# snayfach/MicrobeCensus

Hardware: AMD Instinct MI355X
Metric: reads/sec searched vs marker DB + AGS abs-error, 150 bp @ 1/2/4/8 GPU (higher is better)
Workload: dtype u8/int32

## Files before the change

microbecensus_amd/csrc/k_translate_seg.h:

```cpp
#pragma once
#include "mc_hip_common.h"

#define MC_TS_THREADS 64
#define MC_TS_WAVES (MC_TS_THREADS / 64)
#define MC_TS_READS (MC_TS_THREADS / 6)
#define MC_TS_NLNF(FP) ((FP) + 2 > 24 ? (FP) + 2 : 24)
#define MC_TS_STRIDE(FP) (((((FP) + 76 + 3) >> 2) | 1) << 2)
#define MC_TS_STAGE(L) ((((MC_TS_READS * (L)) > MC_TS_WAVES * 1488 ? (MC_TS_READS * (L)) : MC_TS_WAVES * 1488) + 15) & ~15)

struct McSegWaveLds { unsigned long long best[64]; uint32_t pre[66]; uint32_t pre2[66]; uint32_t bq[64]; uint16_t off[64]; uint8_t n[64]; };
static_assert(sizeof(McHsp) == 48 && sizeof(McGapTask) % 4 == 0, "k_eval_seeds copies its staging buffers as 16- and 4-byte words");
static_assert(sizeof(McSegWaveLds) == 1488, "MC_TS_STAGE reserves 1488 bytes per wave");
#ifdef MC_EXP_TIMING
__device__ unsigned long long g_ts_acc[12], g_ts_cnt[12];
#define MC_TS_TICK(k) do { const unsigned long long now_ = __builtin_readcyclecounter(); if (lane == 0) { ts_acc_[tcat_] += now_ - tlast_; ts_acc_[12 + tcat_] += 1; } tlast_ = now_; tcat_ = (k); } while (0)
#define MC_TS_BEGIN(k) __shared__ unsigned long long ts_acc_[24]; if (lane < 24) ts_acc_[lane] = 0; mc_wave_sync(); unsigned long long tlast_ = __builtin_readcyclecounter(); int tcat_ = (k)
#define MC_TS_PARAMS , unsigned long long &tlast_, int &tcat_, unsigned long long *ts_acc_
#define MC_TS_ARGS , tlast_, tcat_, ts_acc_
#define MC_TS_END do { mc_wave_sync(); if (lane < 12) { atomicAdd(&g_ts_acc[lane], ts_acc_[lane]); atomicAdd(&g_ts_cnt[lane], ts_acc_[12 + lane]); } } while (0)
#else
#define MC_TS_TICK(k) do { } while (0)
#define MC_TS_BEGIN(k) do { } while (0)
#define MC_TS_PARAMS
#define MC_TS_ARGS
#define MC_TS_END do { } while (0)
#endif
#define MC_SEG_KEY_ONE 0xBFF0000000000000ull

__device__ __forceinline__ unsigned long long mc_seg_key(double x)
{
    const unsigned long long u = (unsigned long long)__double_as_longlong(x);
    return (u >> 63) ? ~u : (u | 0x8000000000000000ull);
}

__device__ __forceinline__ void mc_seg_wave(const double *lnf, const int32_t *fx, const uint64_t *__restrict__ segtab, uint8_t *prot, int n, bool act, const McSegWS ws, McSegWaveLds *WL,
                                         const uint8_t *lds0, int lane MC_TS_PARAMS)
{
    const int W = (n <= 11) ? 8 : 12;
    MC_TS_TICK(0);
    enum { POP = 0, SCAN = 1, WAIT = 2, DONE = 3 };
    int st = (act && W <= n) ? POP : DONE;
    McBits192 Flo, Fhi, lo, nhi, mk;
    mc_bits_clear(Flo); mc_bits_clear(Fhi); mc_bits_clear(lo); mc_bits_clear(nhi); mc_bits_clear(mk);
    if (st != DONE) {
        mc_seg_window_flags_rg(fx, prot, n, W, Flo, Fhi);
        if (!(Flo.a | Flo.b | Flo.c)) st = DONE;
    }
    int sp = 1, base = 0, m = 0, i = 0, lowlim = 0, loi = 0, hii = 0;
    bool any = false;
    if (st != DONE) ws.stk[0] = (int16_t)(uint16_t)(n << 8);
    const unsigned long long ltmask = (1ull << lane) - 1;
    for (;;) {
        MC_TS_TICK(1);
        while (st == POP || st == SCAN) {
            if (st == POP) {
                if (sp == 0) { st = DONE; break; }
                sp--;
                base = MC_SEG_START(ws.stk[sp]); m = MC_SEG_LEN(ws.stk[sp]);
                if (W > m) continue;
                lo = mc_seg_flags_of(Flo, base, m, W);
                i = mc_bits_next(lo, 0);
                if (i >= m) continue;
                nhi = mc_bits_andnot(mc_bits_low(m), mc_seg_flags_of(Fhi, base, m, W));
                lowlim = 0; st = SCAN;
            }
            loi = mc_bits_prev(nhi, i) + 1; if (loi < lowlim) loi = lowlim;
            hii = mc_bits_next(nhi, i) - 1; if (hii > m - 1) hii = m - 1;
            st = WAIT;
        }
        const unsigned long long req = __ballot(st == WAIT);
        MC_TS_TICK(2);
        if (req == 0) break;
        const int nreq = __popcll(req);
        const int myr = __popcll(req & ltmask);
        const int myn = hii - loi + 1;
        if (st == WAIT) {
            WL->off[myr] = (uint16_t)((prot + base + loi) - lds0);
            WL->n[myr] = (uint8_t)myn;
            WL->best[myr] = MC_SEG_KEY_ONE; WL->bq[myr] = 0xFFFFFFFFu;
        }
        mc_wave_sync();
#define MC_SEG_CJ(j, sh) (((((j) >> (sh)) * (((j) >> (sh)) + 1)) << (sh)) / 2 + ((j) & ((1 << (sh)) - 1)) * (((j) >> (sh)) + 1))
        int sh0 = 3, sh1 = 3;
        {
            int K = 0, j0 = 0;
            if (lane < nreq) { const int nn = WL->n[lane], minlen = (nn - 100 > 1) ? nn - 100 : 1; K = nn - minlen; j0 = nn - 15 > 0 ? (nn - 15 < K ? nn - 15 : K) : 0; }
            uint32_t s0 = 0, s1 = 0;
#pragma unroll
            for (int sh = 2; sh >= 0; sh--) {
                const uint32_t c1 = (uint32_t)MC_SEG_CJ(j0, sh), c0 = (uint32_t)MC_SEG_CJ(K, sh) - c1;
                const uint32_t t0 = (uint32_t)__builtin_amdgcn_readlane((int)mc_wave_scan_add(c0), 63), t1 = (uint32_t)__builtin_amdgcn_readlane((int)mc_wave_scan_add(c1), 63);
                if (t0 <= 64) sh0 = sh;
                if (t1 <= 64) sh1 = sh;
            }
            {
                const uint32_t c1 = sh1 == 0 ? (uint32_t)MC_SEG_CJ(j0, 0) : sh1 == 1 ? (uint32_t)MC_SEG_CJ(j0, 1) : sh1 == 2 ? (uint32_t)MC_SEG_CJ(j0, 2) : (uint32_t)MC_SEG_CJ(j0, 3);
                const uint32_t cj0 = sh0 == 0 ? (uint32_t)MC_SEG_CJ(j0, 0) : sh0 == 1 ? (uint32_t)MC_SEG_CJ(j0, 1) : sh0 == 2 ? (uint32_t)MC_SEG_CJ(j0, 2) : (uint32_t)MC_SEG_CJ(j0, 3);
                const uint32_t ck = sh0 == 0 ? (uint32_t)MC_SEG_CJ(K, 0) : sh0 == 1 ? (uint32_t)MC_SEG_CJ(K, 1) : sh0 == 2 ? (uint32_t)MC_SEG_CJ(K, 2) : (uint32_t)MC_SEG_CJ(K, 3);
                s0 = mc_wave_scan_add(ck - cj0); s1 = mc_wave_scan_add(c1);
            }
            if (lane == 0) { WL->pre[0] = 0; WL->pre2[0] = 0; }
            WL->pre[lane + 1] = s0; WL->pre2[lane + 1] = s1;
        }
        mc_wave_sync();
        for (int cls = 0; cls < 2; cls++) {
        const uint32_t *pre = cls ? WL->pre2 : WL->pre;
        const uint32_t total = pre[nreq];
        const int sh = cls ? sh1 : sh0, R = 1 << sh;
        for (uint32_t p0 = 0; p0 < total; p0 += 64) {
            MC_TS_TICK(3 + cls);
            const uint32_t p = p0 + (uint32_t)lane;
            const bool ok = p < total;
            int r = 0;
            for (int stp = 32; stp > 0; stp >>= 1) { const int k = r + stp; if (k < nreq && p >= pre[k]) r = k; }
            if (!ok) r = 0;
            const int nn = WL->n[r];
            int x = (int)(p - pre[r]);
            if (cls == 0) { const int minlen = (nn - 100 > 1) ? nn - 100 : 1, K = nn - minlen, j0 = nn - 15 > 0 ? (nn - 15 < K ? nn - 15 : K) : 0; x += MC_SEG_CJ(j0, sh); }
            int A = (int)((sqrtf(1.0f + 8.0f * (float)x / (float)R) - 1.0f) * 0.5f);
            while ((((A + 1) * (A + 2)) << sh) / 2 <= x) A++;
            while (((A * (A + 1)) << sh) / 2 > x) A--;
            const int rem = x - ((A * (A + 1)) << sh) / 2, B = rem / (A + 1), run = rem - B * (A + 1);
            const int j = (A << sh) + B, wfirst = run << sh, wlast = (wfirst + R - 1 < j) ? wfirst + R - 1 : j;
            const uint8_t *s = lds0 + WL->off[r];
            const int len = nn - j;
            const uint32_t qbase = (uint32_t)(j * (j + 1) / 2);
            unsigned long long key = MC_SEG_KEY_ONE;
            uint32_t kq = 0xFFFFFFFFu;
            if (ok) {
                if (cls == 0) {
                    McRhState rg; rg.clo = 0; rg.chi = 0; rg.hist = 0;
                    for (int k = 0; k < len; k++) mc_rh_add(rg, s[wfirst + k]);
                    const int cnt = wlast - wfirst + 1;
                    uint64_t svs[8];
#pragma unroll
                    for (int t = 0; t < 8; t++) {
                        svs[t] = rg.hist | ((uint64_t)len << 60);
                        if (t + 1 < cnt) { mc_rh_remove(rg, s[wfirst + t]); mc_rh_add(rg, s[wfirst + t + len]); }
                    }
#pragma unroll
                    for (int t0 = 0; t0 < 8; t0 += 4) {
                        if (t0 && R <= 4) break;
                        ulonglong2 ea[4], eb[4];
#pragma unroll
                        for (int t = 0; t < 4; t++) {
// ... 28 lines not shown
            mc_wave_sync();
            const unsigned long long nb = WL->best[r];
            if (ok && nb != old) WL->bq[r] = 0xFFFFFFFFu;
            mc_wave_sync();
            if (cand && key == nb) atomicMin(&WL->bq[r], kq);
            mc_wave_sync();
        }
        }
#undef MC_SEG_CJ
        MC_TS_TICK(6);
        if (st == WAIT) {
            const uint32_t q = WL->bq[myr];
            int lend = 0, rend = myn - 1;
            if (q != 0xFFFFFFFFu) {
                int j = (int)((sqrtf((float)(8u * q + 1u)) - 1.0f) * 0.5f);
                while ((uint32_t)((j + 1) * (j + 2) / 2) <= q) j++;
                while ((uint32_t)(j * (j + 1) / 2) > q) j--;
                const int len = myn - j, w0 = (int)q - j * (j + 1) / 2;
                lend = w0; rend = len + w0 - 1;
            }
            const int leftend = loi + lend, rightend = hii - (myn - rend - 1);
            if (i < leftend) {
                const int l2 = loi, r2 = leftend - 1;
                sp = mc_seg_push(ws.stk, sp, W, base + l2, r2 - l2 + 1);
            }
            mk = mc_bits_or(mk, mc_bits_range(base + leftend, base + rightend));
            any = true;
            lowlim = ((hii < rightend) ? hii : rightend) + 1;
            i = mc_bits_next(lo, lowlim);
            st = i < m ? SCAN : POP;
        }
        mc_wave_sync();
    }
    MC_TS_TICK(7);
    if (any) for (int k = 0; k < n; k++) if (mc_bits_test(mk, k)) prot[k] = MC_INV;
    MC_TS_TICK(10);
}

__device__ __forceinline__ int mc_translate_frame_lds(const uint8_t *cod, const uint8_t *read, int len, int frame, uint8_t *prot)
{
    const int o = frame % 3;
    int n = (len - o) / 3;
    if (n < 0) n = 0;
    const bool rc = frame >= 3;
    const uint32_t set = rc ? MC_NT_RC_SET : MC_NT_FWD_SET, perm = rc ? MC_NT_RC_PERM : MC_NT_FWD_PERM;
    const uint8_t *p = read + (rc ? len - 1 - o : o);
    const int s = rc ? -1 : 1;
    int i = 0;
    for (; i + 8 <= n; i += 8) {
        uint32_t b[24], w[2] = {0, 0};
#pragma unroll
        for (int k = 0; k < 24; k++) b[k] = p[s * (3 * i + k)];
#pragma unroll
        for (int k = 0; k < 8; k++) {
            const int a0 = mc_nt_code(b[3 * k], set, perm), a1 = mc_nt_code(b[3 * k + 1], set, perm), a2 = mc_nt_code(b[3 * k + 2], set, perm);
            const uint32_t aa = cod[(16 * a0 + 4 * a1 + a2) & 63];
            w[k >> 2] |= ((a0 | a1 | a2) < 0 ? (uint32_t)MC_INV : aa) << (8 * (k & 3));
        }
        *(uint32_t *)(prot + i) = w[0];
        *(uint32_t *)(prot + i + 4) = w[1];
    }
    for (; i < n; i++) {
        const int a0 = mc_nt_code(p[s * (3 * i)], set, perm), a1 = mc_nt_code(p[s * (3 * i + 1)], set, perm), a2 = mc_nt_code(p[s * (3 * i + 2)], set, perm);
        const uint8_t aa = cod[(16 * a0 + 4 * a1 + a2) & 63];
        prot[i] = (a0 | a1 | a2) < 0 ? (uint8_t)MC_INV : aa;
    }
    return n;
}

template <bool STAGED>
__global__ void __attribute__((amdgpu_waves_per_eu(4, 4))) __launch_bounds__(MC_TS_THREADS) k_translate_seg(const McTables *__restrict__ T, const uint8_t *__restrict__ reads, int L,
                                                       int64_t nreads, uint8_t *__restrict__ frames, int FP, const uint64_t *__restrict__ segtab)
{
    extern __shared__ __attribute__((aligned(16))) uint8_t smem[];
    const int tid = threadIdx.x;
    const int64_t r0 = (int64_t)blockIdx.x * MC_TS_READS;
    const int nr = (int)((nreads - r0) < MC_TS_READS ? (nreads - r0) : MC_TS_READS);
    const int rbytes = nr * L;
    const int stride = MC_TS_STRIDE(FP);
    __shared__ int32_t fxs[64];
#ifdef MC_EXP_TIMING
    const int lane = mc_lane();
#endif
    MC_TS_BEGIN(8);
    uint8_t *sreads = smem;
    const int nlnf = MC_TS_NLNF(FP);
    double *lnf = (double *)(smem + (STAGED ? MC_TS_STAGE(L) : MC_TS_STAGE(0)));
    uint8_t *rows = (uint8_t *)(lnf + nlnf);
    __shared__ __attribute__((aligned(4))) uint8_t cod[64];
    if (tid < 64) fxs[tid] = T->seg_dout[tid];
    if (tid < 16) ((uint32_t *)cod)[tid] = ((const uint32_t *)T->codon)[tid];
    for (int i = tid; i < nlnf; i += MC_TS_THREADS) lnf[i] = T->lnfac[i];
    if (STAGED) {
        const uint8_t *src = reads + r0 * L;
        const int head = (int)((4 - ((uintptr_t)src & 3)) & 3), nhead = head < rbytes ? head : rbytes;
        if (tid < nhead) sreads[tid] = src[tid];
        const int nw = (rbytes - nhead) >> 2;
        if (nhead == 0) for (int i = tid; i < nw; i += MC_TS_THREADS) ((uint32_t *)sreads)[i] = ((const uint32_t *)src)[i];
        else for (int i = tid; i < nw; i += MC_TS_THREADS) { const uint32_t w = ((const uint32_t *)(src + nhead))[i]; uint8_t *d = sreads + nhead + 4 * i; d[0] = (uint8_t)w; d[1] = (uint8_t)(w >> 8); d[2] = (uint8_t)(w >> 16); d[3] = (uint8_t)(w >> 24); }
        for (int i = nhead + 4 * nw + tid; i < rbytes; i += MC_TS_THREADS) sreads[i] = src[i];
    }
    __syncthreads();
    MC_TS_TICK(9);
    const int lr = tid / 6, f = tid - lr * 6;
    uint8_t *prot = rows + (size_t)tid * stride;
    int n = 0;
    if (lr < nr) n = mc_translate_frame_lds(cod, STAGED ? sreads + lr * L : reads + (r0 + lr) * L, L, f, prot);
    __syncthreads();
    {
        McSegWS ws; ws.comp = prot + FP; ws.sv = prot + FP + 20; ws.stk = (int16_t *)(prot + FP + 44);
        mc_seg_wave(lnf, fxs, segtab, prot, n, lr < nr, ws, (McSegWaveLds *)smem + (tid >> 6), rows, mc_lane() MC_TS_ARGS);
        if (lr < nr) for (int i = n; i < FP; i++) prot[i] = MC_INV;
    }
    __syncthreads();
    {
        uint32_t *dst = (uint32_t *)(frames + r0 * 6 * FP);
        const int total = nr * 6 * FP / 4, fpw = FP / 4;
        for (int i = tid; i < total; i += MC_TS_THREADS) { const int row = i / fpw, col = i - row * fpw; dst[i] = *(const uint32_t *)(rows + (size_t)row * stride + 4 * col); }
    }
    MC_TS_TICK(0);
    MC_TS_END;
}
```

microbecensus_amd/csrc/mc_hip.hip:

```cpp
#include "mc_hip_common.h"
#include "k_translate_seg.h"
#include "k_enumerate.h"
#include "k_eval_seeds.h"
#include "k_gapped.h"
#include "k_order.h"
#include "k_finish.h"
#include "k_grid.h"
#include "k_simulate.h"
#include "k_community.h"
#include "k_varlen.h"
#include "k_classes.h"
#include "k_bootstrap.h"
#include "k_wfit.h"
#include "mc_pieces.h"
#include "mc_ahead.h"
#include "mc_owned.h"
#include "mc_abund.h"

#include <map>

struct McCtx {
    McStream stream; hipStream_t side = nullptr, side2 = nullptr;
    McEvent ev[8], ev_fork, ev_join, ev_join2;
    int64_t cap_reads = 0; int pool_len = 0;
    int ts_staged = -1;
    uint32_t cap_tasks = 0, cap_gaps = 0, cap_hsps = 0, cap_rows = 0;
    McDev<uint8_t> d_frames_base; uint8_t *d_frames = nullptr;
    McDev<unsigned long long> d_stats;
    McDev<McSeedTask> d_tasks; McDev<McGapTask> d_gaps; McDev<McHsp> d_hsps, d_v, d_tmp;
    McDev<uint64_t> d_k64, d_hkeys, d_hplace, d_places; McDev<uint32_t> d_idx, d_idxo, d_heads, d_scan, d_gsz, d_nv, d_ghist;
    McDev<uint32_t> d_counters;
    McDev<McRow> d_rows; McDev<uint32_t> d_nrow, d_rowoff; McDev<McBestHit> d_best, d_bestof; McDev<uint8_t> d_low, d_cand;
    McDev<McGapCell> d_gws_full; McDev<uint32_t> d_retry, d_retry2; int gap_threads_full = 0;
    McDev<unsigned long long> d_gtab; uint32_t gtab_slots = 0; McDev<uint32_t> d_gleader; McDev<McFlankOut> d_fout;
    McPin<uint32_t> h_c; McPin<unsigned long long> h_stats; McPin<McBestHit> h_best; size_t h_best_cap = 0;
    const uint8_t *reads = nullptr; int64_t n = 0, first_read_id = 0, first = 0;
    int ahead_from = -1;
    bool own_a0 = true;
    uint32_t ntasks = 0, ngaps = 0, gpad = 0, nh = 0, nh_all = 0, nheads = 0, nrows = 0, nbest = 0, nsegs = 0;
    bool busy = false;
};

struct mc_handle {
    McHostIndex H;
    std::vector<int32_t> fam;
    int nfam = 0, device = 0;
    McDev<uint8_t> d_res_base; uint8_t *d_res = nullptr; McDev<uint32_t> d_off, d_bstart, d_post; McDev<unsigned long long> d_post8; McDev<uint16_t> d_keys; McDev<int32_t> d_fam;
    McDev<McTables> d_T; McDev<McClassPars> d_P;
    McTables hT; McClassPars hP;
    int read_len = 0, FP = 0; bool run_set = false;
    McDev<uint32_t> d_bitmap;
    McDev<McBucketRec> d_rec;
    McDev<uint32_t> d_filt, d_wild, d_pair; McDev<uint64_t> d_segtab; McDev<unsigned long long> d_rt;
    bool fast_enum = false;
    bool count_traffic = false;
    int pipe_nout = 0;
    bool keep_rows = true;
    bool best_only = false;
    bool rows_stay = false;
    float train_ms[3] = {0, 0, 0};
// ... 291 lines not shown
    const int newFP = ((read_len / 3 + 2) + 3) & ~3;
    if (newFP != h->FP || read_len != h->read_len) h->ctx.cap_reads = 0;
    h->read_len = read_len; h->FP = newFP; h->run_set = true;
    h->cls_set = false;
    MC_OT("set_run: segtab, uploads", t0);
    return 0;
}

static void best_materialize(mc_handle *h);
static int ensure_capacity(mc_handle *h, McCtx &c, int64_t nreads)
{
    if (nreads <= c.cap_reads && h->read_len <= c.pool_len) return 0;
    if (h->best_from == &c) best_materialize(h);
    ahead_drop(h);
    double t0 = mc_now();
    int64_t cap = nreads;
    if (cap > (1 << 21) - 1) { g_err = "batch larger than 2097151 reads"; return -1; }
    const int64_t L = h->read_len;
    c.cap_reads = 0;
    c.cap_tasks = (uint32_t)std::min<int64_t>(cap * (L + 32) + (1 << 20) + (int64_t)256 * 32 * MC_EN_BLK, 0x7fffffff);
    const int64_t ev_pad = (int64_t)256 * 8 * (MC_EV_BS / 64) * MC_EV_BLK;
    c.cap_gaps = (uint32_t)std::min<int64_t>(cap * (L / 8 + 8) + (1 << 18) + ev_pad, (1 << 27) - 2);
    c.cap_hsps = (uint32_t)std::min<int64_t>(cap * (L / 3 + 8) + (1 << 20) + ev_pad, 0x7fffffff);
    c.cap_rows = (uint32_t)std::min<int64_t>(cap * 16 + (1 << 20), 0x7fffffff);
    c.gap_threads_full = 16 * 1024;
    if (c.d_frames_base.alloc((size_t)cap * 6 * h->FP + 128) || c.d_tasks.alloc(c.cap_tasks) ||
        c.d_gaps.alloc(c.cap_gaps) || c.d_hsps.alloc(c.cap_hsps) || c.d_v.alloc(c.cap_hsps) ||
        c.d_tmp.alloc((size_t)c.cap_hsps * 2) || c.d_k64.alloc(c.cap_hsps) || c.d_hkeys.alloc(c.cap_hsps) || c.d_hplace.alloc(c.cap_hsps) || c.d_places.alloc(c.cap_hsps) || c.d_idx.alloc(c.cap_hsps) ||
        c.d_idxo.alloc(c.cap_hsps) || c.d_heads.alloc((size_t)cap + 2) || c.d_scan.alloc((size_t)4100) || c.d_gsz.alloc(c.cap_hsps) || c.d_nv.alloc((size_t)cap + 1) || c.d_rows.alloc(c.cap_rows) ||
        c.d_low.alloc((size_t)cap + 64) || c.d_cand.alloc((size_t)cap + 64) || c.d_nrow.alloc((size_t)cap + 1) || c.d_rowoff.alloc((size_t)cap + 1) || c.d_best.alloc((size_t)cap + 1) || c.d_bestof.alloc((size_t)cap + 1) ||
        c.d_gws_full.alloc((size_t)c.gap_threads_full * MC_GAP_W) || c.d_retry.alloc((size_t)c.cap_gaps * 2 + (size_t)cap + 1) || c.d_retry2.alloc((size_t)c.cap_gaps * 2) || c.d_gleader.alloc((size_t)c.cap_gaps) ||
        c.d_fout.alloc((size_t)c.cap_gaps * 2))
        return -1;
    c.d_frames = c.d_frames_base + 64;
    HIPCK(hipMemsetAsync(c.d_frames_base, MC_INV, 64, c.stream));
    if (c.h_best.alloc((size_t)cap + 1)) return -1;
    c.h_best_cap = (size_t)cap + 1;
    c.cap_reads = cap; c.pool_len = (int)L;
    HIPCK(hipStreamSynchronize(c.stream));
    MC_OT("ensure_capacity (pools)", t0);
    return 0;
}

static int reads_reserve(mc_handle *h, int64_t nreads)
{
    const int64_t need = nreads * (int64_t)h->read_len + 16;
    if (need > h->cap_own) { reads_change(h); if (h->d_reads.alloc((size_t)need)) return -1; h->cap_own = need; }
    return 0;
}

extern "C" int mc_upload(mc_handle *h, const uint8_t *reads, int64_t nreads)
{
    if (!h || !h->run_set) { g_err = "mc_set_run() must be called first"; return -1; }
    HIPCK(hipSetDevice(h->device));
    reads_change(h);
    if (reads_reserve(h, nreads)) return -1;
    if (nreads) HIPCK(hipMemcpyAsync(h->d_reads, reads, (size_t)nreads * h->read_len, hipMemcpyHostToDevice, h->ctx.stream));
    HIPCK(hipStreamSynchronize(h->ctx.stream));
    h->reads_dev = h->d_reads; h->nreads = nreads;
    return 0;
}

extern "C" int mc_attach(mc_handle *h, const void *device_reads, int64_t nreads)
{
    if (!h || !h->run_set) { g_err = "mc_set_run() must be called first"; return -1; }
    reads_change(h);
    h->reads_dev = (const uint8_t *)device_reads; h->nreads = nreads;
    return 0;
}

static int stage_wait(McCtx &c) { HIPCK(hipStreamSynchronize(c.stream)); return 0; }
static int counters_to_host(McCtx &c) { HIPCK(hipMemcpyAsync(c.h_c, c.d_counters, sizeof(uint32_t) * C_N, hipMemcpyDeviceToHost, c.stream)); return 0; }

#ifdef MC_EXP_TIMING
static int exp_timing_dump(mc_handle *h, McCtx &c, char stage)
{
    ahead_drop(h);
    if (stage == 'a') {
        HIPCK(hipStreamSynchronize(c.stream));
        unsigned long long acc[12], cnt[12];
        HIPCK(hipMemcpyFromSymbol(acc, HIP_SYMBOL(g_ts_acc), sizeof acc)); HIPCK(hipMemcpyFromSymbol(cnt, HIP_SYMBOL(g_ts_cnt), sizeof cnt));
        const char *nm[12] = {"flags", "advance", "numbering", "class-0 rounds", "class-1 rounds", "reduction", "owners", "mask", "staging", "translation", "write-out", ""};
        const double waves = (double)((c.n + MC_TS_READS - 1) / MC_TS_READS) * MC_TS_WAVES;
        for (int k = 0; k < 11; k++) fprintf(stderr, "ts-timing %-15s %9.1f cycles/wave  %8.2f entries/wave  total %8.1f Mcycles\n", nm[k], (double)acc[k] / waves, (double)cnt[k] / waves, acc[k] / 1e6);
        unsigned long long z[12] = {0, 0, 0, 0, 0, 0, 0, 0, 0, 0, 0, 0};
        HIPCK(hipMemcpyToSymbol(HIP_SYMBOL(g_ts_acc), z, sizeof z)); HIPCK(hipMemcpyToSymbol(HIP_SYMBOL(g_ts_cnt), z, sizeof z));
    } else {
        HIPCK(hipStreamSynchronize(c.stream)); HIPCK(hipStreamSynchronize(c.side));
        unsigned long long acc[8], cnt[8];
        HIPCK(hipMemcpyFromSymbol(acc, HIP_SYMBOL(g_fh_acc), sizeof acc)); HIPCK(hipMemcpyFromSymbol(cnt, HIP_SYMBOL(g_fh_cnt), sizeof cnt));
        {
            unsigned long long fr[8];
            HIPCK(hipMemcpyFromSymbol(fr, HIP_SYMBOL(g_fr_acc), sizeof fr));
            const char *fn[7] = {"groups", "items", "std::sort", "threshold, keys", "heap sort", "rows", "classification"};
            for (int k = 0; k < 7; k++) fprintf(stderr, "fr-timing %-17s total %9.1f Mcycles (thread wall time, summed)\n", fn[k], fr[k] / 1e6);
            unsigned long long z8[8] = {0, 0, 0, 0, 0, 0, 0, 0};
            HIPCK(hipMemcpyToSymbol(HIP_SYMBOL(g_fr_acc), z8, sizeof z8));
            HIPCK(hipMemcpyFromSymbol(fr, HIP_SYMBOL(g_fr_acc2), sizeof fr));
            const char *gn[8] = {"-", "sort by frame", "sort by start, stable", "choice", "sum statistics", "copies", "groups (count)", "groups linked (count)"};
            for (int k = 1; k < 8; k++) fprintf(stderr, "fg-timing %-22s %12.1f M\n", gn[k], fr[k] / 1e6);
            HIPCK(hipMemcpyToSymbol(HIP_SYMBOL(g_fr_acc2), z8, sizeof z8));
        }
        {
            unsigned long long ev[8];
            HIPCK(hipMemcpyFromSymbol(ev, HIP_SYMBOL(g_ev_acc), sizeof ev));
            const char *en[7] = {"loop, records asked", "survivors queued", "X-drop extension", "HSP, marks", "records written", "residue wait + seed", "growth, gate"};
            for (int k = 0; k < 7; k++) fprintf(stderr, "ev-timing %-21s total %9.1f Mcycles (lane 0 of every wave)\n", en[k], ev[k] / 1e6);
            unsigned long long z8[8] = {0, 0, 0, 0, 0, 0, 0, 0};
            HIPCK(hipMemcpyToSymbol(HIP_SYMBOL(g_ev_acc), z8, sizeof z8));
            unsigned long long tr[4];
            HIPCK(hipMemcpyFromSymbol(tr, HIP_SYMBOL(g_ev_turns), sizeof tr));
            fprintf(stderr, "ev-turns forward: %.1f M lane-turns in %.2f M wave-turns = %.1f lanes of 64; backward: %.1f M in %.2f M = %.1f lanes\n", tr[0] / 1e6, tr[1] / 1e6, tr[1] ? (double)tr[0] / (double)tr[1] : 0.0,
                    tr[2] / 1e6, tr[3] / 1e6, tr[3] ? (double)tr[2] / (double)tr[3] : 0.0);
            HIPCK(hipMemcpyToSymbol(HIP_SYMBOL(g_ev_turns), z8, sizeof tr));
        }
        const char *nm[8] = {"group starts", "groups", "scan, items", "sort", "threshold, ranks", "heap sort", "rows", "other"};
        for (int k = 0; k < 8; k++) fprintf(stderr, "fh-timing %-17s total %9.1f Mcycles %9llu entries\n", nm[k], acc[k] / 1e6, cnt[k]);
        {
            unsigned long long w[12];
            HIPCK(hipMemcpyFromSymbol(w, HIP_SYMBOL(g_fh_worst), sizeof w));
            fprintf(stderr, "fh-worst read: %llu stacked HSPs, %.3f Mcycles:", w[0] & 0xFFFFF, (double)(w[0] >> 20) / 1e6);
            for (int k = 0; k < 8; k++) fprintf(stderr, " %s %.3f", nm[k], (double)w[1 + k] / 1e6);
            fprintf(stderr, "\n");
            unsigned long long z12[12] = {0, 0, 0, 0, 0, 0, 0, 0, 0, 0, 0, 0};
            HIPCK(hipMemcpyToSymbol(HIP_SYMBOL(g_fh_worst), z12, sizeof z12));
        }
        unsigned long long z[8] = {0, 0, 0, 0, 0, 0, 0, 0};
        HIPCK(hipMemcpyToSymbol(HIP_SYMBOL(g_fh_acc), z, sizeof z)); HIPCK(hipMemcpyToSymbol(HIP_SYMBOL(g_fh_cnt), z, sizeof z));
    }
    return 0;
}
#else
static int exp_timing_dump(mc_handle *, McCtx &, char) { return 0; }
#endif

static int stage_a0(mc_handle *h, McCtx &c, hipStream_t st, const uint8_t *reads, int64_t at, int64_t n, hipEvent_t e0, hipEvent_t e1)
{
    const int L = h->read_len, FP = h->FP;
    uint8_t *frames = c.d_frames + at * 6 * FP;
    HIPCK(hipEventRecord(e0, st));
    const size_t lds_rest = (size_t)MC_TS_NLNF(FP) * 8 + (size_t)MC_TS_THREADS * MC_TS_STRIDE(FP);
    const size_t lds_staged = (size_t)MC_TS_STAGE(L) + lds_rest, lds_direct = (size_t)MC_TS_STAGE(0) + lds_rest;
    static const int ts_force = getenv("MC_TS_STAGED") ? atoi(getenv("MC_TS_STAGED")) : -1;
    const size_t cu_lds = 160 * 1024 - 1024;
    const bool staged = ts_force >= 0 ? ts_force != 0 : cu_lds / lds_staged >= cu_lds / lds_direct;
    const size_t lds = staged ? lds_staged : lds_direct;
    c.ts_staged = staged ? 1 : 0;
    const unsigned ts_blocks = (unsigned)((n + MC_TS_READS - 1) / MC_TS_READS);
    if (staged) {
        if (lds > 48 * 1024) HIPCK(hipFuncSetAttribute((const void *)k_translate_seg<true>, hipFuncAttributeMaxDynamicSharedMemorySize, (int)lds));
        k_translate_seg<true><<<dim3(ts_blocks), dim3(MC_TS_THREADS), lds, st>>>(h->d_T, reads, L, n, frames, FP, h->d_segtab);
    } else {
        if (lds > 48 * 1024) HIPCK(hipFuncSetAttribute((const void *)k_translate_seg<false>, hipFuncAttributeMaxDynamicSharedMemorySize, (int)lds));
        k_translate_seg<false><<<dim3(ts_blocks), dim3(MC_TS_THREADS), lds, st>>>(h->d_T, reads, L, n, frames, FP, h->d_segtab);
    }
    HIPCK(hipEventRecord(e1, st));
    return 0;
}

static int stage_a(mc_handle *h, McCtx &c, int64_t covered)
{
    const int64_t n = c.n;
    const int L = h->read_len, FP = h->FP;
    hipStream_t st = c.stream;
    McIndex X = dev_index(h);
    c.ntasks = c.ngaps = c.gpad = c.nh = c.nheads = c.nrows = c.nbest = c.nsegs = 0;
    HIPCK(hipMemsetAsync(c.d_counters, 0, sizeof(uint32_t) * C_N, st));
    HIPCK(hipMemsetAsync(c.d_stats, 0, sizeof(unsigned long long) * S_N, st));
    if (h->best_only) HIPCK(hipMemsetAsync(c.d_cand, 0, (size_t)n, st));
    HIPCK(hipMemsetAsync(c.d_low, 0, (size_t)n, st));
    c.own_a0 = covered < n;
    if (!c.own_a0) HIPCK(hipEventRecord(c.ev[1], st));
    else if (stage_a0(h, c, st, c.reads + covered * L, covered, n - covered, c.ev[0], c.ev[1])) return -1;
    if (exp_timing_dump(h, c, 'a')) return -1;
    const int64_t threads = n * 6;
    if (h->fast_enum) {
        const bool enq = !h->count_traffic;
        const size_t per_wave = enq ? MC_ENQ_WAVE_LDS(FP, L) : sizeof(McEnWave) + MC_EN_WAVE_LDS(FP, L);
        int waves = 0, bpc = 1;
        {
            static const int shapes_q[][2] = {{8, 2}, {4, 4}, {16, 1}, {12, 1}, {4, 3}, {8, 1}, {4, 2}, {4, 1}};
            static const int shapes_c[][2] = {{12, 2}, {8, 3}, {4, 6}, {4, 5}, {16, 1}, {8, 2}, {4, 4}, {12, 1}, {4, 3}, {8, 1}, {4, 2}, {4, 1}};
            if (enq) { for (const auto &sh : shapes_q) if (!waves && (size_t)sh[1] * (64 + sh[0] * per_wave) <= 160 * 1024) { waves = sh[0]; bpc = sh[1]; } }
            else for (const auto &sh : shapes_c) if (!waves && (size_t)sh[1] * (64 + sh[0] * per_wave) <= 160 * 1024) { waves = sh[0]; bpc = sh[1]; }
        }
        if (!waves) { g_err = "reads too long for the seed kernel's LDS layout"; return -1; }
        const size_t lds2 = 64 + waves * per_wave;
#define MC_LAUNCH_EN(KERNEL, WV)                                                                                                                   \
// ... 309 lines not shown

extern "C" int mc_range_begin(mc_handle *h, int64_t first, int64_t count, int64_t first_read_id)
{
    if (range_check(h, first, count)) return -1;
    if (count <= 0) { g_err = "mc_range_begin: an empty range"; return -1; }
    if (h->pipe_nout) { g_err = "mc_range_begin: a range is in flight already (mc_range_end first)"; return -1; }
    const int rc = range_begin(h, h->ctx, first, count, first_read_id);
    if (rc) return rc;
    h->pipe_nout = 1;
    return 0;
}

static int range_end_next(mc_handle *h, int64_t first, int64_t count, bool predict)
{
    if (predict) count = mc_ahead_predict(h->ctx.first, h->ctx.n, h->nreads, &first);
    return range_end(h, h->ctx, first, count);
}

extern "C" int64_t mc_ranges_translated_ahead(const mc_handle *h) { return h ? h->ahead_used : 0; }

extern "C" int mc_range_end(mc_handle *h)
{
    if (!h) { g_err = "null handle"; return -1; }
    if (h->pipe_nout == 0) { g_err = "mc_range_end: no range in flight"; return -1; }
    HIPCK(hipSetDevice(h->device));
    h->pipe_nout = 0;
    return range_end_next(h, 0, 0, true);
}

extern "C" int mc_ranges_in_flight(const mc_handle *h) { return h ? h->pipe_nout : 0; }

extern "C" int64_t mc_debug_stage(mc_handle *h, int what, void *dst, int64_t cap_bytes, int32_t *record_bytes)
{
    if (!h || !h->run_set || what < 0 || what > 5) { g_err = "mc_debug_stage: bad argument"; return -1; }
    if (h->pipe_nout) { g_err = "mc_debug_stage: ranges are in flight"; return -1; }
    HIPCK(hipSetDevice(h->device));
    ahead_drop(h);
    const McCtx &c = h->ctx;
    if (what == 4) {
        if (!c.h_c) { g_err = "mc_debug_stage: no range has run"; return -1; }
        const uint32_t v[3] = {c.h_c[C_ITEMS], c.h_c[C_RETRY], c.h_c[C_RETRY2]};
        if (record_bytes) *record_bytes = (int32_t)sizeof(uint32_t);
        if (dst && (int64_t)sizeof v <= cap_bytes) memcpy(dst, v, sizeof v);
        return (int64_t)sizeof v;
    }
    if (what == 5) {
        if (c.ts_staged < 0) { g_err = "mc_debug_stage: no range has run"; return -1; }
        const uint32_t v = (uint32_t)c.ts_staged;
        if (record_bytes) *record_bytes = (int32_t)sizeof v;
        if (dst && (int64_t)sizeof v <= cap_bytes) memcpy(dst, &v, sizeof v);
        return (int64_t)sizeof v;
    }
    const void *src = nullptr; int64_t bytes = 0; int32_t rec = 0;
    if (what == 0) { src = c.d_frames; rec = h->FP; bytes = c.n * 6 * (int64_t)h->FP; }
    else if (what == 1) { src = c.d_tasks; rec = (int32_t)sizeof(McSeedTask); bytes = (int64_t)c.ntasks * rec; }
    else if (what == 2) { src = c.d_gaps; rec = (int32_t)sizeof(McGapTask); bytes = (int64_t)c.ngaps * rec; }
    else { src = c.d_hsps; rec = (int32_t)sizeof(McHsp); bytes = (int64_t)(c.nh_all + (c.h_c ? c.h_c[C_HPAD] : 0u)) * rec; }
    if (record_bytes) *record_bytes = rec;
    if (dst && bytes && bytes <= cap_bytes) { HIPCK(hipStreamSynchronize(c.stream)); HIPCK(hipMemcpy(dst, src, (size_t)bytes, hipMemcpyDeviceToHost)); }
    return bytes;
}

extern "C" int mc_set_counting(mc_handle *h, int on)
{
    if (!h) { g_err = "null handle"; return -1; }
    ahead_drop(h);
    h->count_traffic = on != 0;
    return 0;
}

extern "C" int mc_run(mc_handle *h, int64_t first_read_id) { return h ? mc_run_range(h, 0, h->nreads, first_read_id) : -1; }

#define MC_STREAM_BATCH 2000000
static int64_t stream_batch()
{
    if (const char *e = getenv("MC_STREAM_BATCH")) { const long long v = atoll(e); if (v >= 1000 && v <= MC_STREAM_BATCH) return (int64_t)v; }
    return MC_STREAM_BATCH;
}
struct McBatchSlot { uint8_t *pin = nullptr, *dev = nullptr; int64_t n = 0, first = 0; int state = 0;  int64_t rc = 0; };

static int run_stream(mc_handle *h, const std::function<int64_t(uint8_t *, int64_t, int64_t *)> &fetch, int64_t first_read_id, int64_t expect_reads = 0)
{
    HIPCK(hipSetDevice(h->device));
// ... 1388 lines not shown
```

Before: 66.29 million.

## Split SEG masking into front pass plus compacted work-list trim pass with refill

The translate kernel now only translates frames and computes SEG window flags, writing frames out and recording which frames actually need low-complexity trimming into per-block slots. A scan plus list kernel compacts those frame ids, and a second launch of the kernel processes only the flagged frames. Each wave keeps lanes busy by refilling idle lanes with new frames from chunked work ranges, instead of idling once its own reads finish. This aims to remove the lane and wave imbalance of the per-read SEG loop, at the cost of extra launches, a flags buffer in global memory and a second frame round trip for trimmed frames.

```diff
diff --git a/microbecensus_amd/csrc/k_translate_seg.h b/microbecensus_amd/csrc/k_translate_seg.h
--- a/microbecensus_amd/csrc/k_translate_seg.h
+++ b/microbecensus_amd/csrc/k_translate_seg.h
@@ -12,18 +12,21 @@
 static_assert(sizeof(McHsp) == 48 && sizeof(McGapTask) % 4 == 0, "k_eval_seeds copies its staging buffers as 16- and 4-byte words");
 static_assert(sizeof(McSegWaveLds) == 1488, "MC_TS_STAGE reserves 1488 bytes per wave");
 #ifdef MC_EXP_TIMING
-__device__ unsigned long long g_ts_acc[12], g_ts_cnt[12];
-#define MC_TS_TICK(k) do { const unsigned long long now_ = __builtin_readcyclecounter(); if (lane == 0) { ts_acc_[tcat_] += now_ - tlast_; ts_acc_[12 + tcat_] += 1; } tlast_ = now_; tcat_ = (k); } while (0)
-#define MC_TS_BEGIN(k) __shared__ unsigned long long ts_acc_[24]; if (lane < 24) ts_acc_[lane] = 0; mc_wave_sync(); unsigned long long tlast_ = __builtin_readcyclecounter(); int tcat_ = (k)
+#define MC_TS_NCAT 16
+__device__ unsigned long long g_ts_acc[2][MC_TS_NCAT], g_ts_cnt[2][MC_TS_NCAT];
+#define MC_TS_TICK(k) do { const unsigned long long now_ = __builtin_readcyclecounter(); if (lane == 0) { ts_acc_[tcat_] += now_ - tlast_; ts_acc_[MC_TS_NCAT + tcat_] += 1; } tlast_ = now_; tcat_ = (k); } while (0)
+#define MC_TS_COUNT(k, v) do { if (lane == 0) { ts_acc_[k] += (unsigned long long)(v); ts_acc_[MC_TS_NCAT + (k)] += 1; } } while (0)
+#define MC_TS_BEGIN(k) __shared__ unsigned long long ts_acc_[2 * MC_TS_NCAT]; if (lane < 2 * MC_TS_NCAT) ts_acc_[lane] = 0; mc_wave_sync(); unsigned long long tlast_ = __builtin_readcyclecounter(); int tcat_ = (k)
 #define MC_TS_PARAMS , unsigned long long &tlast_, int &tcat_, unsigned long long *ts_acc_
 #define MC_TS_ARGS , tlast_, tcat_, ts_acc_
-#define MC_TS_END do { mc_wave_sync(); if (lane < 12) { atomicAdd(&g_ts_acc[lane], ts_acc_[lane]); atomicAdd(&g_ts_cnt[lane], ts_acc_[12 + lane]); } } while (0)
+#define MC_TS_END(pass) do { mc_wave_sync(); if (lane < MC_TS_NCAT) { atomicAdd(&g_ts_acc[pass][lane], ts_acc_[lane]); atomicAdd(&g_ts_cnt[pass][lane], ts_acc_[MC_TS_NCAT + lane]); } } while (0)
 #else
 #define MC_TS_TICK(k) do { } while (0)
+#define MC_TS_COUNT(k, v) do { } while (0)
 #define MC_TS_BEGIN(k) do { } while (0)
 #define MC_TS_PARAMS
 #define MC_TS_ARGS
-#define MC_TS_END do { } while (0)
+#define MC_TS_END(pass) do { } while (0)
 #endif
 #define MC_SEG_KEY_ONE 0xBFF0000000000000ull
 
@@ -33,23 +36,32 @@
     return (u >> 63) ? ~u : (u | 0x8000000000000000ull);
 }
 
-__device__ __forceinline__ void mc_seg_wave(const double *lnf, const int32_t *fx, const uint64_t *__restrict__ segtab, uint8_t *prot, int n, bool act, const McSegWS ws, McSegWaveLds *WL,
-                                         const uint8_t *lds0, int lane MC_TS_PARAMS)
-{
-    const int W = (n <= 11) ? 8 : 12;
-    MC_TS_TICK(0);
-    enum { POP = 0, SCAN = 1, WAIT = 2, DONE = 3 };
-    int st = (act && W <= n) ? POP : DONE;
+#ifndef MC_SEG_CHUNK
+#define MC_SEG_CHUNK 128
+#endif
+#ifndef MC_SEG_REFILL
+#define MC_SEG_REFILL 24
+#endif
+struct McSegTake { const uint32_t *list; uint32_t total; };
+
+__device__ __forceinline__ void mc_seg_wave(const double *lnf, const uint64_t *__restrict__ segtab, uint8_t *prot, const McSegWS ws, McSegWaveLds *WL,
+                                         uint8_t *lds0, int lane, const McSegTake tk, uint8_t *frames, const uint32_t *__restrict__ flags, int wps, int L, int FP, int stride MC_TS_PARAMS)
+{
+    enum { POP = 0, SCAN = 1, WAIT = 2, DONE = 3, EMPTY = 4, NEW = 5 };
+    int st = EMPTY, n = 0, W = 8;
+    uint32_t fid = 0;
     McBits192 Flo, Fhi, lo, nhi, mk;
     mc_bits_clear(Flo); mc_bits_clear(Fhi); mc_bits_clear(lo); mc_bits_clear(nhi); mc_bits_clear(mk);
-    if (st != DONE) {
-        mc_seg_window_flags_rg(fx, prot, n, W, Flo, Fhi);
-        if (!(Flo.a | Flo.b | Flo.c)) st = DONE;
-    }
     int sp = 1, base = 0, m = 0, i = 0, lowlim = 0, loi = 0, hii = 0;
     bool any = false;
-    if (st != DONE) ws.stk[0] = (int16_t)(uint16_t)(n << 8);
     const unsigned long long ltmask = (1ull << lane) - 1;
+    const int fpw = FP / 4;
+    uint32_t *frames32 = (uint32_t *)frames;
+    const uint32_t G = gridDim.x;
+    uint32_t wpos = blockIdx.x * (uint32_t)MC_SEG_CHUNK < tk.total ? blockIdx.x * (uint32_t)MC_SEG_CHUNK : tk.total;
+    uint32_t wend = wpos + MC_SEG_CHUNK < tk.total ? wpos + MC_SEG_CHUNK : tk.total;
+    uint32_t pend = blockIdx.x + G;
+    bool dry = false;
     for (;;) {
         MC_TS_TICK(1);
         while (st == POP || st == SCAN) {
@@ -69,8 +81,67 @@
             st = WAIT;
         }
         const unsigned long long req = __ballot(st == WAIT);
+        {
+            const unsigned long long idle = __ballot(st >= DONE);
+            if (req == 0 || (!(dry && wpos >= wend) && __popcll(idle) >= MC_SEG_REFILL)) {
+                MC_TS_TICK(7);
+                if (st == DONE && any) for (int k = 0; k < n; k++) if (mc_bits_test(mk, k)) prot[k] = MC_INV;
+                MC_TS_TICK(10);
+                const unsigned long long dm = __ballot(st == DONE);
+                if (st == DONE) { const int d = __popcll(dm & ltmask); WL->pre[d] = fid; WL->pre2[d] = (uint32_t)lane; st = EMPTY; }
+                mc_wave_sync();
+                for (int x = lane, nx = __popcll(dm) * fpw; x < nx; x += 64) {
+                    const int e = x / fpw, col = x - e * fpw;
+                    frames32[(size_t)WL->pre[e] * fpw + col] = *(const uint32_t *)(lds0 + (size_t)WL->pre2[e] * stride + 4 * col);
+                }
+                mc_wave_sync();
+                MC_TS_TICK(11);
+                const int nidle = __popcll(idle), myi = __popcll(idle & ltmask);
+                int got = 0;
+                while (got < nidle) {
+                    if (wpos >= wend) {
+                        if (dry) break;
+                        const unsigned long long b = (unsigned long long)pend * MC_SEG_CHUNK;
+                        if (b >= tk.total) { dry = true; break; }
+                        wpos = (uint32_t)b; wend = wpos + MC_SEG_CHUNK < tk.total ? wpos + MC_SEG_CHUNK : tk.total;
+                        pend += G;
+                    }
+                    const int k = nidle - got < (int)(wend - wpos) ? nidle - got : (int)(wend - wpos);
+                    if (st == EMPTY && myi >= got && myi < got + k) { fid = tk.list[wpos + (uint32_t)(myi - got)]; st = NEW; }
+                    wpos += (uint32_t)k; got += k;
+                }
+                const unsigned long long nm = __ballot(st == NEW);
+                if (nm) {
+                    if (st == NEW) { const int e = __popcll(nm & ltmask); WL->pre[e] = fid; WL->pre2[e] = (uint32_t)lane; }
+                    mc_wave_sync();
+                    for (int x = lane, nx = __popcll(nm) * fpw; x < nx; x += 64) {
+                        const int e = x / fpw, col = x - e * fpw;
+                        *(uint32_t *)(lds0 + (size_t)WL->pre2[e] * stride + 4 * col) = frames32[(size_t)WL->pre[e] * fpw + col];
+                    }
+                    mc_wave_sync();
+                    uint32_t *fl = (uint32_t *)(prot + FP);
+                    for (int x = lane, nx = __popcll(nm) * 2 * wps; x < nx; x += 64) {
+                        const int e = x / (2 * wps), col = x - e * 2 * wps;
+                        ((uint32_t *)(lds0 + (size_t)WL->pre2[e] * stride + FP))[col] = flags[(size_t)WL->pre[e] * (2 * wps) + col];
+                    }
+                    mc_wave_sync();
+                    if (st == NEW) {
+                        const int f = (int)(fid % 6u);
+                        n = (L - f % 3) / 3; W = (n <= 11) ? 8 : 12;
+                        st = DONE; any = false; sp = 1; mc_bits_clear(mk);
+                        uint32_t v[10];
+#pragma unroll
+                        for (int w = 0; w < 5; w++) { v[w] = w < wps ? fl[w] : 0u; v[5 + w] = w < wps ? fl[wps + w] : 0u; }
+                        Flo.a = v[0] | ((uint64_t)v[1] << 32); Flo.b = v[2] | ((uint64_t)v[3] << 32); Flo.c = v[4];
+                        Fhi.a = v[5] | ((uint64_t)v[6] << 32); Fhi.b = v[7] | ((uint64_t)v[8] << 32); Fhi.c = v[9];
+                        if (W <= n && (Flo.a | Flo.b | Flo.c)) { st = POP; ws.stk[0] = (int16_t)(uint16_t)(n << 8); }
+                    }
+                    continue;
+                }
+                if (req == 0) break;
+            }
+        }
         MC_TS_TICK(2);
-        if (req == 0) break;
         const int nreq = __popcll(req);
         const int myr = __popcll(req & ltmask);
         const int myn = hii - loi + 1;
@@ -103,14 +174,17 @@
             WL->pre[lane + 1] = s0; WL->pre2[lane + 1] = s1;
         }
         mc_wave_sync();
+        MC_TS_COUNT(13, (WL->pre[nreq] + 63) / 64 + (WL->pre2[nreq] + 63) / 64);
         for (int cls = 0; cls < 2; cls++) {
         const uint32_t *pre = cls ? WL->pre2 : WL->pre;
         const uint32_t total = pre[nreq];
         const int sh = cls ? sh1 : sh0, R = 1 << sh;
+        if (total) MC_TS_COUNT(14 + cls, R);
         for (uint32_t p0 = 0; p0 < total; p0 += 64) {
             MC_TS_TICK(3 + cls);
             const uint32_t p = p0 + (uint32_t)lane;
             const bool ok = p < total;
+            MC_TS_COUNT(12, total - p0 < 64 ? total - p0 : 64);
             int r = 0;
             for (int stp = 32; stp > 0; stp >>= 1) { const int k = r + stp; if (k < nreq && p >= pre[k]) r = k; }
             if (!ok) r = 0;
@@ -205,8 +279,6 @@
         }
         mc_wave_sync();
     }
-    MC_TS_TICK(7);
-    if (any) for (int k = 0; k < n; k++) if (mc_bits_test(mk, k)) prot[k] = MC_INV;
     MC_TS_TICK(10);
 }
 
@@ -241,29 +313,34 @@
     return n;
 }
 
+struct McTsArgs {
+    const McTables *T; const uint8_t *reads; int L; int64_t nreads; uint8_t *frames; int FP; const uint64_t *segtab;
+    uint32_t *slots, *cnt;
+    uint32_t *flags; int wps;
+    const uint32_t *list; uint32_t *ctl;
+};
+#define MC_TS_SLOTS (MC_TS_READS * 6)
+#define MC_TS_WPS(FP) ((FP) - 13 + 31 >= 32 ? ((FP) - 13 + 31) / 32 : 1)
+
 template <bool STAGED>
-__global__ void __attribute__((amdgpu_waves_per_eu(4, 4))) __launch_bounds__(MC_TS_THREADS) k_translate_seg(const McTables *__restrict__ T, const uint8_t *__restrict__ reads, int L,
-                                                       int64_t nreads, uint8_t *__restrict__ frames, int FP, const uint64_t *__restrict__ segtab)
+__device__ __forceinline__ void mc_ts_front(const McTsArgs &a)
 {
     extern __shared__ __attribute__((aligned(16))) uint8_t smem[];
+    const McTables *__restrict__ T = a.T; const uint8_t *__restrict__ reads = a.reads;
+    const int L = a.L, FP = a.FP;
     const int tid = threadIdx.x;
     const int64_t r0 = (int64_t)blockIdx.x * MC_TS_READS;
-    const int nr = (int)((nreads - r0) < MC_TS_READS ? (nreads - r0) : MC_TS_READS);
+    const int nr = (int)((a.nreads - r0) < MC_TS_READS ? (a.nreads - r0) : MC_TS_READS);
     const int rbytes = nr * L;
     const int stride = MC_TS_STRIDE(FP);
     __shared__ int32_t fxs[64];
-#ifdef MC_EXP_TIMING
     const int lane = mc_lane();
-#endif
     MC_TS_BEGIN(8);
     uint8_t *sreads = smem;
-    const int nlnf = MC_TS_NLNF(FP);
-    double *lnf = (double *)(smem + (STAGED ? MC_TS_STAGE(L) : MC_TS_STAGE(0)));
-    uint8_t *rows = (uint8_t *)(lnf + nlnf);
+    uint8_t *rows = smem + (STAGED ? MC_TS_STAGE(L) : MC_TS_STAGE(0)) + (size_t)MC_TS_NLNF(FP) * 8;
     __shared__ __attribute__((aligned(4))) uint8_t cod[64];
     if (tid < 64) fxs[tid] = T->seg_dout[tid];
     if (tid < 16) ((uint32_t *)cod)[tid] = ((const uint32_t *)T->codon)[tid];
-    for (int i = tid; i < nlnf; i += MC_TS_THREADS) lnf[i] = T->lnfac[i];
     if (STAGED) {
         const uint8_t *src = reads + r0 * L;
         const int head = (int)((4 - ((uintptr_t)src & 3)) & 3), nhead = head < rbytes ? head : rbytes;
@@ -279,18 +356,73 @@
     uint8_t *prot = rows + (size_t)tid * stride;
     int n = 0;
     if (lr < nr) n = mc_translate_frame_lds(cod, STAGED ? sreads + lr * L : reads + (r0 + lr) * L, L, f, prot);
+    MC_TS_TICK(0);
+    bool need = false;
+    {
+        const int W = (n <= 11) ? 8 : 12;
+        if (lr < nr && W <= n) {
+            McBits192 Flo, Fhi;
+            mc_bits_clear(Flo); mc_bits_clear(Fhi);
+            mc_seg_window_flags_rg(fxs, prot, n, W, Flo, Fhi);
+            need = (Flo.a | Flo.b | Flo.c) != 0;
+            if (need) {
+                uint32_t *d = a.flags + ((size_t)(r0 * 6) + (size_t)tid) * (size_t)(2 * a.wps);
+                const uint32_t vl[5] = {(uint32_t)Flo.a, (uint32_t)(Flo.a >> 32), (uint32_t)Flo.b, (uint32_t)(Flo.b >> 32), (uint32_t)Flo.c};
+                const uint32_t vh[5] = {(uint32_t)Fhi.a, (uint32_t)(Fhi.a >> 32), (uint32_t)Fhi.b, (uint32_t)(Fhi.b >> 32), (uint32_t)Fhi.c};
+#pragma unroll
+                for (int w = 0; w < 5; w++) if (w < a.wps) { d[w] = vl[w]; d[a.wps + w] = vh[w]; }
+            }
+        }
+        if (lr < nr) for (int i = n; i < FP; i++) prot[i] = MC_INV;
+    }
+    MC_TS_TICK(10);
+    {
+        const unsigned long long nm = __ballot(need);
+        if (need) a.slots[(size_t)blockIdx.x * MC_TS_SLOTS + (uint32_t)__popcll(nm & ((1ull << lane) - 1))] = (uint32_t)(r0 * 6) + (uint32_t)tid;
+        if (lane == 0) a.cnt[blockIdx.x] = (uint32_t)__popcll(nm);
+    }
     __syncthreads();
     {
-        McSegWS ws; ws.comp = prot + FP; ws.sv = prot + FP + 20; ws.stk = (int16_t *)(prot + FP + 44);
-        mc_seg_wave(lnf, fxs, segtab, prot, n, lr < nr, ws, (McSegWaveLds *)smem + (tid >> 6), rows, mc_lane() MC_TS_ARGS);
-        if (lr < nr) for (int i = n; i < FP; i++) prot[i] = MC_INV;
-    }
-    __syncthreads();
-    {
-        uint32_t *dst = (uint32_t *)(frames + r0 * 6 * FP);
+        uint32_t *dst = (uint32_t *)(a.frames + r0 * 6 * FP);
         const int total = nr * 6 * FP / 4, fpw = FP / 4;
         for (int i = tid; i < total; i += MC_TS_THREADS) { const int row = i / fpw, col = i - row * fpw; dst[i] = *(const uint32_t *)(rows + (size_t)row * stride + 4 * col); }
     }
     MC_TS_TICK(0);
-    MC_TS_END;
-}
+    MC_TS_END(0);
+}
+
+__device__ __forceinline__ void mc_ts_trim(const McTsArgs &a)
+{
+    extern __shared__ __attribute__((aligned(16))) uint8_t smem[];
+    const int FP = a.FP, tid = threadIdx.x;
+    McSegTake tk; tk.list = a.list; tk.total = a.ctl[0];
+    if (tk.total == 0) return;
+    const int stride = MC_TS_STRIDE(FP);
+    const int lane = mc_lane();
+    MC_TS_BEGIN(8);
+    const int nlnf = MC_TS_NLNF(FP);
+    double *lnf = (double *)(smem + MC_TS_STAGE(0));
+    uint8_t *rows = (uint8_t *)(lnf + nlnf);
+    for (int i = tid; i < nlnf; i += MC_TS_THREADS) lnf[i] = a.T->lnfac[i];
+    __syncthreads();
+    uint8_t *prot = rows + (size_t)tid * stride;
+    McSegWS ws; ws.comp = prot + FP; ws.sv = prot + FP + 20; ws.stk = (int16_t *)(prot + FP + 44);
+    mc_seg_wave(lnf, a.segtab, prot, ws, (McSegWaveLds *)smem, rows, lane, tk, a.frames, a.flags, a.wps, a.L, FP, stride MC_TS_ARGS);
+    MC_TS_END(1);
+}
+
+template <int PASS>
+__global__ void __attribute__((amdgpu_waves_per_eu(4, 4))) __launch_bounds__(MC_TS_THREADS) k_translate_seg(const McTsArgs a)
+{
+    if constexpr (PASS == 2) mc_ts_trim(a); else mc_ts_front<PASS == 1>(a);
+}
+
+__global__ void __launch_bounds__(256) k_translate_seg_list(const uint32_t *__restrict__ slots, const uint32_t *__restrict__ cnt, const uint32_t *__restrict__ off, uint32_t nblocks,
+                                                           uint32_t *__restrict__ list, uint32_t *__restrict__ ctl)
+{
+    const uint32_t i = blockIdx.x * 256u + threadIdx.x, b = i >> 6, k = i & 63u;
+    if (b >= nblocks) return;
+    const uint32_t c = cnt[b], o = off[b];
+    if (k < c) list[o + k] = slots[(size_t)b * MC_TS_SLOTS + k];
+    if (b == nblocks - 1 && k == 0) ctl[0] = o + c;
+}
diff --git a/microbecensus_amd/csrc/mc_hip.hip b/microbecensus_amd/csrc/mc_hip.hip
--- a/microbecensus_amd/csrc/mc_hip.hip
+++ b/microbecensus_amd/csrc/mc_hip.hip
@@ -24,8 +24,10 @@
     McEvent ev[8], ev_fork, ev_join, ev_join2;
     int64_t cap_reads = 0; int pool_len = 0;
     int ts_staged = -1;
+    uint32_t trim_blocks = 0;
     uint32_t cap_tasks = 0, cap_gaps = 0, cap_hsps = 0, cap_rows = 0;
     McDev<uint8_t> d_frames_base; uint8_t *d_frames = nullptr;
+    McDev<uint32_t> d_seg_slots, d_seg_cnt, d_seg_off, d_seg_list, d_seg_ctl, d_seg_sums, d_seg_flags;
     McDev<unsigned long long> d_stats;
     McDev<McSeedTask> d_tasks; McDev<McGapTask> d_gaps; McDev<McHsp> d_hsps, d_v, d_tmp;
     McDev<uint64_t> d_k64, d_hkeys, d_hplace, d_places; McDev<uint32_t> d_idx, d_idxo, d_heads, d_scan, d_gsz, d_nv, d_ghist;
@@ -383,6 +385,12 @@
         c.d_gws_full.alloc((size_t)c.gap_threads_full * MC_GAP_W) || c.d_retry.alloc((size_t)c.cap_gaps * 2 + (size_t)cap + 1) || c.d_retry2.alloc((size_t)c.cap_gaps * 2) || c.d_gleader.alloc((size_t)c.cap_gaps) ||
         c.d_fout.alloc((size_t)c.cap_gaps * 2))
         return -1;
+    {
+        const size_t wgs = (size_t)(cap + MC_TS_READS - 1) / MC_TS_READS;
+        if (c.d_seg_slots.alloc(wgs * MC_TS_SLOTS + 1) || c.d_seg_cnt.alloc(wgs + 1) || c.d_seg_off.alloc(wgs + 1) || c.d_seg_list.alloc((size_t)cap * 6 + 1) || c.d_seg_flags.alloc((size_t)cap * 6 * 2 * MC_TS_WPS(h->FP) + 1) ||
+            c.d_seg_ctl.alloc(1) || c.d_seg_sums.alloc(wgs / MC_SCAN_BLK + 2))
+            return -1;
+    }
     c.d_frames = c.d_frames_base + 64;
     HIPCK(hipMemsetAsync(c.d_frames_base, MC_INV, 64, c.stream));
     if (c.h_best.alloc((size_t)cap + 1)) return -1;
@@ -429,12 +437,17 @@
     ahead_drop(h);
     if (stage == 'a') {
         HIPCK(hipStreamSynchronize(c.stream));
-        unsigned long long acc[12], cnt[12];
+        unsigned long long acc[2][MC_TS_NCAT], cnt[2][MC_TS_NCAT];
         HIPCK(hipMemcpyFromSymbol(acc, HIP_SYMBOL(g_ts_acc), sizeof acc)); HIPCK(hipMemcpyFromSymbol(cnt, HIP_SYMBOL(g_ts_cnt), sizeof cnt));
-        const char *nm[12] = {"flags", "advance", "numbering", "class-0 rounds", "class-1 rounds", "reduction", "owners", "mask", "staging", "translation", "write-out", ""};
+        const char *nm[12] = {"flags", "advance", "numbering", "class-0 rounds", "class-1 rounds", "reduction", "owners", "mask", "staging, tables", "translation", "write-out", "refill"};
         const double waves = (double)((c.n + MC_TS_READS - 1) / MC_TS_READS) * MC_TS_WAVES;
-        for (int k = 0; k < 11; k++) fprintf(stderr, "ts-timing %-15s %9.1f cycles/wave  %8.2f entries/wave  total %8.1f Mcycles\n", nm[k], (double)acc[k] / waves, (double)cnt[k] / waves, acc[k] / 1e6);
-        unsigned long long z[12] = {0, 0, 0, 0, 0, 0, 0, 0, 0, 0, 0, 0};
+        for (int p = 0; p < 2; p++)
+            for (int k = 0; k < 12; k++)
+                if (cnt[p][k]) fprintf(stderr, "ts-timing pass %d %-15s %9.1f cycles/wave  %8.2f entries/wave  total %8.1f Mcycles\n", p + 1, nm[k], (double)acc[p][k] / waves, (double)cnt[p][k] / waves, acc[p][k] / 1e6);
+        const char *cn[4] = {"items per round", "rounds per batch", "R per batch, <= 15", "R per batch, > 15"};
+        for (int k = 0; k < 4; k++)
+            if (cnt[1][12 + k]) fprintf(stderr, "ts-timing pass 2 %-18s %8.2f  over %10llu\n", cn[k], (double)acc[1][12 + k] / (double)cnt[1][12 + k], cnt[1][12 + k]);
+        unsigned long long z[2][MC_TS_NCAT] = {};
         HIPCK(hipMemcpyToSymbol(HIP_SYMBOL(g_ts_acc), z, sizeof z)); HIPCK(hipMemcpyToSymbol(HIP_SYMBOL(g_ts_cnt), z, sizeof z));
     } else {
         HIPCK(hipStreamSynchronize(c.stream)); HIPCK(hipStreamSynchronize(c.side));
@@ -490,6 +503,7 @@
     const int L = h->read_len, FP = h->FP;
     uint8_t *frames = c.d_frames + at * 6 * FP;
     HIPCK(hipEventRecord(e0, st));
+    if (n <= 0) { HIPCK(hipEventRecord(e1, st)); return 0; }
     const size_t lds_rest = (size_t)MC_TS_NLNF(FP) * 8 + (size_t)MC_TS_THREADS * MC_TS_STRIDE(FP);
     const size_t lds_staged = (size_t)MC_TS_STAGE(L) + lds_rest, lds_direct = (size_t)MC_TS_STAGE(0) + lds_rest;
     static const int ts_force = getenv("MC_TS_STAGED") ? atoi(getenv("MC_TS_STAGED")) : -1;
@@ -498,13 +512,24 @@
     const size_t lds = staged ? lds_staged : lds_direct;
     c.ts_staged = staged ? 1 : 0;
     const unsigned ts_blocks = (unsigned)((n + MC_TS_READS - 1) / MC_TS_READS);
+    McTsArgs a;
+    a.T = h->d_T; a.reads = reads; a.L = L; a.nreads = n; a.frames = frames; a.FP = FP; a.segtab = h->d_segtab;
+    a.slots = c.d_seg_slots; a.cnt = c.d_seg_cnt; a.list = c.d_seg_list; a.ctl = c.d_seg_ctl;
+    a.flags = c.d_seg_flags + (size_t)at * 6 * 2 * MC_TS_WPS(FP); a.wps = MC_TS_WPS(FP);
     if (staged) {
-        if (lds > 48 * 1024) HIPCK(hipFuncSetAttribute((const void *)k_translate_seg<true>, hipFuncAttributeMaxDynamicSharedMemorySize, (int)lds));
-        k_translate_seg<true><<<dim3(ts_blocks), dim3(MC_TS_THREADS), lds, st>>>(h->d_T, reads, L, n, frames, FP, h->d_segtab);
+        if (lds > 48 * 1024) HIPCK(hipFuncSetAttribute((const void *)k_translate_seg<1>, hipFuncAttributeMaxDynamicSharedMemorySize, (int)lds));
+        k_translate_seg<1><<<dim3(ts_blocks), dim3(MC_TS_THREADS), lds, st>>>(a);
     } else {
-        if (lds > 48 * 1024) HIPCK(hipFuncSetAttribute((const void *)k_translate_seg<false>, hipFuncAttributeMaxDynamicSharedMemorySize, (int)lds));
-        k_translate_seg<false><<<dim3(ts_blocks), dim3(MC_TS_THREADS), lds, st>>>(h->d_T, reads, L, n, frames, FP, h->d_segtab);
-    }
+        if (lds > 48 * 1024) HIPCK(hipFuncSetAttribute((const void *)k_translate_seg<0>, hipFuncAttributeMaxDynamicSharedMemorySize, (int)lds));
+        k_translate_seg<0><<<dim3(ts_blocks), dim3(MC_TS_THREADS), lds, st>>>(a);
+    }
+    if (mc_scan_u32(c.d_seg_cnt, ts_blocks, c.d_seg_off, c.d_seg_sums, st)) return -1;
+    k_translate_seg_list<<<dim3((ts_blocks * 64u + 255u) / 256u), dim3(256), 0, st>>>(c.d_seg_slots, c.d_seg_cnt, c.d_seg_off, ts_blocks, c.d_seg_list, c.d_seg_ctl);
+    static const int trim_cap = getenv("MC_SEG_TRIM_WAVES") ? atoi(getenv("MC_SEG_TRIM_WAVES")) : 0;
+    const unsigned trim_blocks = trim_cap > 0 ? (unsigned)trim_cap : (unsigned)((n * 6 + MC_SEG_CHUNK - 1) / MC_SEG_CHUNK);
+    c.trim_blocks = trim_blocks;
+    if (lds_direct > 48 * 1024) HIPCK(hipFuncSetAttribute((const void *)k_translate_seg<2>, hipFuncAttributeMaxDynamicSharedMemorySize, (int)lds_direct));
+    k_translate_seg<2><<<dim3(trim_blocks), dim3(MC_TS_THREADS), lds_direct, st>>>(a);
     HIPCK(hipEventRecord(e1, st));
     return 0;
 }
@@ -880,7 +905,7 @@
 
 extern "C" int64_t mc_debug_stage(mc_handle *h, int what, void *dst, int64_t cap_bytes, int32_t *record_bytes)
 {
-    if (!h || !h->run_set || what < 0 || what > 5) { g_err = "mc_debug_stage: bad argument"; return -1; }
+    if (!h || !h->run_set || what < 0 || what > 6) { g_err = "mc_debug_stage: bad argument"; return -1; }
     if (h->pipe_nout) { g_err = "mc_debug_stage: ranges are in flight"; return -1; }
     HIPCK(hipSetDevice(h->device));
     ahead_drop(h);
@@ -897,6 +922,13 @@
         const uint32_t v = (uint32_t)c.ts_staged;
         if (record_bytes) *record_bytes = (int32_t)sizeof v;
         if (dst && (int64_t)sizeof v <= cap_bytes) memcpy(dst, &v, sizeof v);
+        return (int64_t)sizeof v;
+    }
+    if (what == 6) {
+        if (c.ts_staged < 0) { g_err = "mc_debug_stage: no range has run"; return -1; }
+        uint32_t v[2] = {0, c.trim_blocks};
+        if (record_bytes) *record_bytes = (int32_t)sizeof(uint32_t);
+        if (dst && (int64_t)sizeof v <= cap_bytes) { HIPCK(hipStreamSynchronize(c.stream)); HIPCK(hipMemcpy(&v[0], c.d_seg_ctl, sizeof(uint32_t), hipMemcpyDeviceToHost)); memcpy(dst, v, sizeof v); }
         return (int64_t)sizeof v;
     }
     const void *src = nullptr; int64_t bytes = 0; int32_t rec = 0;
```

Measured after the change: 66.83 million (median of 6 runs). No clear change (+0.8%).
